# vshmyhlo/retinanet-tensorflow

Measured on AMD Instinct MI355X. Metric: train images/sec (MobileNetV2-FPN RetinaNet 512x512, bs=2/GPU), higher is better.
Workload: dtype f32

## Files before the change

### include/rn_hip.h

```cpp
#ifndef RN_HIP_H
#define RN_HIP_H

#include <stddef.h>
#include <stdint.h>

#ifdef __cplusplus
extern "C" {
#endif

typedef void* rn_stream_t;

enum rn_status {
  RN_OK = 0,
  RN_EINVAL = -1,
  RN_EUNSUPPORTED = -2,
  RN_EHIP = -3,
  RN_EWORKSPACE = -4
};

enum rn_act { RN_ACT_NONE = 0, RN_ACT_RELU = 1, RN_ACT_ELU = 2, RN_ACT_RELU6 = 3, RN_ACT_SIGMOID = 4 };
enum rn_loss_mode { RN_LOSS_BCE_DICE = 0, RN_LOSS_FOCAL = 1 };
enum rn_opt { RN_OPT_MOMENTUM = 0, RN_OPT_RMSPROP = 1, RN_OPT_ADAM = 2 };

#define RN_MAX_SEG 16

typedef struct rn_reduce_list rn_reduce_list;

#define RN_API_VERSION 411
int rn_version(void);
const char* rn_last_error(void);

void rn_same_pad(int n, int k, int s, int* out, int* pad_before);

typedef struct rn_conv_seg {
  const float* x;
  const float* wgt;
  const float* bias;
  float* y;
  const float* dy;
  float* dx;
  int32_t n, h, w;
  int32_t cout;
  int32_t x_ld;
  int32_t x_coff;
  int64_t wgt_bytes;
} rn_conv_seg;

typedef struct rn_conv_geom {
  int32_t kh, kw, stride, cin;
  int32_t groups;
} rn_conv_geom;
// ... 220 lines not shown

size_t rn_resize_pair_u8_augment_batch_workspace(int k, int oh, int ow);
int rn_resize_pair_u8_augment_batch(const uint8_t* raw, int64_t sample_stride_bytes, const rn_augment_desc* desc, int k,
                                    float* pairs, int oh, int ow, const float* mean, const float* stdv, void* workspace,
                                    size_t workspace_bytes, rn_stream_t stream);

typedef struct rn_loss_seg {
  const float* cls_logit;
  const float* cls_label;
  const float* reg_pred;
  const float* reg_label;
  const uint8_t* trainable;
  float* d_cls_logit;
  float* d_reg_pred;
  int64_t rows;
} rn_loss_seg;

#define RN_LOSS_STATS_HEADER 8
size_t rn_loss_workspace(const rn_loss_seg* segs, int nseg, int num_classes);
int rn_loss_fwd(const rn_loss_seg* segs, int nseg, int num_classes, int mode, float* stats, float* class_loss_out,
                float* regr_loss_out, void* workspace, size_t workspace_bytes, rn_stream_t stream);
int rn_loss_bwd(const rn_loss_seg* segs, int nseg, int num_classes, int mode, const float* stats,
                const float* g_cls, const float* g_reg, rn_stream_t stream);

typedef struct rn_wino_gn {
  const float* in_rows;
  const float* in_gamma;
  const float* in_beta;
  int32_t in_groups, in_act;
  float in_eps;
  float* out_rows;
  int32_t out_groups;
  const void* u_ready;
  int32_t urot_ready;
} rn_wino_gn;
size_t rn_wino_gn_rows(const rn_conv_seg* segs, int nseg, int tile);
size_t rn_conv3x3_winograd_gn_u_bytes(int cin, int cout, int tile);
int rn_conv3x3_winograd_gn_weights(const float* w, int cin, int cout, int tile, void* u_out, size_t u_out_bytes, float* urot_out,
                                   rn_stream_t stream);
int rn_conv3x3_winograd_gn(const rn_conv_seg* segs, int nseg, int cin, int cout, const float* w, const float* bias, int tile,
                           const rn_wino_gn* gn, void* workspace, size_t workspace_bytes, float* v_buf, float* urot_buf,
                           rn_stream_t stream);
typedef struct rn_wino_gn_bwd {
  const float* in_rows;
  const float* in_gamma;
  const float* in_beta;
// ... 182 lines not shown
```

### retinanet-tensorflow_amd/_rn.py

```python
import ctypes as C
import os

import torch

_HERE = os.path.dirname(os.path.abspath(__file__))
LIB_PATH = os.environ.get("RN_LIB_PATH") or os.path.join(_HERE, "librn_hip.so")

MAX_SEG = 16
ACT = {None: 0, "none": 0, "linear": 0, "relu": 1, "elu": 2, "relu6": 3, "sigmoid": 4}
LOSS_MODE = {"bce_dice": 0, "focal": 1}
OPT = {"momentum": 0, "rmsprop": 1, "adam": 2}
OPT_BLOCK = 1024
LR_MAX_BOUNDARIES = 8
LOSS_STATS_HEADER = 8
API_VERSION = 411


class RnError(RuntimeError):
    pass


class LrSchedule(C.Structure):
    _fields_ = [("kind", C.c_int32), ("n_boundaries", C.c_int32), ("base_lr", C.c_double), ("warmup_factor", C.c_double),
                ("final_factor", C.c_double), ("decay_factor", C.c_double), ("warmup_steps", C.c_int64), ("total_steps", C.c_int64),
                ("boundaries", C.c_int64 * LR_MAX_BOUNDARIES)]


class ConvSeg(C.Structure):
    _fields_ = [("x", C.c_void_p), ("wgt", C.c_void_p), ("bias", C.c_void_p), ("y", C.c_void_p),
                ("dy", C.c_void_p), ("dx", C.c_void_p),
                ("n", C.c_int32), ("h", C.c_int32), ("w", C.c_int32), ("cout", C.c_int32),
                ("x_ld", C.c_int32), ("x_coff", C.c_int32), ("wgt_bytes", C.c_int64)]


class AssignLevel(C.Structure):
    _fields_ = [("anchor_sizes", C.c_void_p), ("grid_h", C.c_int32), ("grid_w", C.c_int32), ("cls_out", C.c_void_p),
                ("reg_out", C.c_void_p), ("trainable_out", C.c_void_p), ("argmax_out", C.c_void_p)]

# ... 112 lines not shown
class DetParams(C.Structure):
    _fields_ = [("n", C.c_int32), ("num_classes", C.c_int32), ("max_per_class", C.c_int32),
                ("score_threshold", C.c_float), ("iou_threshold", C.c_float), ("max_candidates", C.c_int64)]


_lib = None

SYMBOLS = [
    "rn_version", "rn_last_error", "rn_same_pad",
    "rn_conv2d_fwd_workspace", "rn_conv2d_dgrad_workspace",
    "rn_zero", "rn_conv2d_fwd", "rn_conv2d_stats_rows", "rn_conv2d_fwd_stats", "rn_conv2d_dropout_rows", "rn_conv2d_fwd_dropout", "rn_depthwise_stats_rows", "rn_depthwise_fwd_stats", "rn_group_norm_rows_ok",
    "rn_conv2d_dgrad", "rn_conv2d_wgrad_workspace", "rn_conv2d_wgrad", "rn_conv2d_bwd",
    "rn_conv2d_bias_grad_workspace", "rn_conv2d_bias_grad", "rn_conv3x3_winograd_workspace", "rn_conv3x3_winograd",
    "rn_conv3x3_winograd_wgrad_workspace", "rn_conv3x3_winograd_wgrad", "rn_conv3x3_winograd_keep_bytes",
    "rn_conv3x3_winograd_bwd_workspace", "rn_conv3x3_winograd_bwd", "rn_flush_reductions", "rn_gemm_batched",
    "rn_winograd_bwd_products_workspace", "rn_winograd_bwd_products", "rn_wino_gn_rows", "rn_conv3x3_winograd_gn", "rn_conv3x3_winograd_gn_bwd", "rn_conv3x3_winograd_gn_bwd_wgrad", "rn_reduce_rows", "rn_resize_bilinear_normalize", "rn_resize_pair_u8",
    "rn_resize_pair_u8_augment_workspace", "rn_resize_pair_u8_augment",
    "rn_resize_pair_u8_batch", "rn_resize_pair_u8_augment_batch_workspace", "rn_resize_pair_u8_augment_batch",
    "rn_dwgn_supported", "rn_dwgn_fwd", "rn_dwgn_bwd", "rn_depthwise_fwd", "rn_depthwise_dgrad", "rn_depthwise_wgrad_workspace", "rn_depthwise_wgrad", "rn_depthwise_bwd",
    "rn_group_norm_sync_bytes", "rn_group_norm_workspace", "rn_group_norm_fwd", "rn_group_norm_bwd",
    "rn_act_fwd", "rn_act_bwd", "rn_upsample_add_fwd", "rn_upsample_add_bwd_top",
    "rn_pack_weights_f16", "rn_pack_weights_f16_bytes", "rn_cast_f32_to_f16", "rn_pad_cast_rgb_f16", "rn_conv2d_fwd_f16", "rn_conv2d_f16_fold_rows", "rn_conv2d_fwd_f16_fold", "rn_group_norm_finalize", "rn_group_norm_apply_f16", "rn_group_norm_apply_res_f16", "rn_maxpool_fwd_f16", "rn_maxpool_gn_fwd_f16", "rn_upsample_add_fwd_f16",
    "rn_act_fwd_f16", "rn_flip_width", "rn_dropout", "rn_dropout_strided", "rn_maxpool_fwd", "rn_maxpool_bwd", "rn_maxpool_bwd_arg", "rn_avgpool_fwd", "rn_avgpool_bwd",
    "rn_loss_workspace", "rn_loss_fwd", "rn_loss_bwd",
    "rn_iou", "rn_anchor_assign", "rn_anchor_assign_levels", "rn_anchor_assign_levels_pair", "rn_decode_boxes", "rn_detect_workspace", "rn_detect",
    "rn_boxes_decode", "rn_nms_classwise_workspace", "rn_nms_classwise",
    "rn_optimizer_workspace", "rn_grad_norm_l2reg", "rn_optimizer_step", "rn_counter_add", "rn_add_segs",
    "rn_mb_rows_max", "rn_mb_compact_rows_layout", "rn_mb_compact_rows", "rn_mb_pointwise_rows", "rn_mb_pointwise_fwd", "rn_mb_depthwise_rows", "rn_mb_depthwise_fwd", "rn_mb_apply",
    "rn_mb_resident_sync_bytes", "rn_mb_resident_rows", "rn_mb_resident_fwd", "rn_set_product_mode", "rn_get_product_mode",
    "rn_set_x3_bfrag", "rn_get_x3_bfrag", "rn_x3_bfrag_ok", "rn_x3_bfrag_bytes", "rn_x3_pack_bfrag", "rn_gemm_batched_bfrag", "rn_conv3x3_winograd_gn_u_bytes", "rn_conv3x3_winograd_gn_weights",
    "rn_conv2d_f16_stats_tiles", "rn_group_norm_fwd_f16_tiles",
    "rn_mb_pointwise_bwd_rows", "rn_mb_pointwise_bwd_workspace", "rn_mb_pointwise_bwd",
    "rn_mb_depthwise_bwd_rows", "rn_mb_depthwise_bwd_workspace", "rn_mb_depthwise_bwd",
    "rn_debug_collective_standin", "rn_optimizer_norm_pairs", "rn_optimizer_step_norm", "rn_norm_reg_finalize",
    "rn_lr_schedule_eval", "rn_optimizer_step_norm_lrdev",
]


def lib():
    global _lib
    if _lib is None:
        if not os.path.exists(LIB_PATH):
            raise RnError("librn_hip.so not found at %s: build it with "
                          "`make -C retinanet-tensorflow_amd/csrc` (there is no fallback path)" % LIB_PATH)
        L = C.CDLL(LIB_PATH)
        if not hasattr(L, "rn_version") or L.rn_version() != API_VERSION:
            raise RnError("%s reports ABI version %s, these bindings need %d: rebuild it (make -C retinanet-tensorflow_amd/csrc)"
# ... 110 lines not shown
        L.rn_conv2d_fwd_f16_fold.argtypes = [C.c_void_p, C.c_int, C.c_void_p, C.c_void_p, C.c_void_p]
        L.rn_group_norm_finalize.argtypes = [C.c_void_p, C.c_int, C.c_int, C.c_int, C.c_int, C.c_int, C.c_float, C.c_void_p, C.c_void_p, C.c_void_p]
        L.rn_group_norm_apply_f16.argtypes = [C.c_void_p, C.c_void_p, C.c_void_p, C.c_int, C.c_int, C.c_int, C.c_int, C.c_void_p, C.c_void_p,
                                              C.c_void_p, C.c_void_p, C.c_int, C.c_int, C.c_void_p]
        L.rn_group_norm_apply_res_f16.argtypes = [C.c_void_p, C.c_void_p, C.c_void_p, C.c_void_p, C.c_int, C.c_int, C.c_int, C.c_int, C.c_void_p,
                                                  C.c_void_p, C.c_void_p, C.c_void_p, C.c_int, C.c_int, C.c_void_p]
        L.rn_maxpool_fwd_f16.argtypes = [C.c_void_p] * 2 + [C.c_int] * 6 + [C.c_void_p]
        L.rn_maxpool_gn_fwd_f16.argtypes = [C.c_void_p] * 2 + [C.c_int] * 6 + [C.c_void_p] * 4 + [C.c_int] * 2 + [C.c_void_p]
        L.rn_upsample_add_fwd_f16.argtypes = [C.c_void_p] * 3 + [C.c_int] * 6 + [C.c_void_p]
        L.rn_act_fwd_f16.argtypes = [C.c_void_p, C.c_void_p, C.c_int64, C.c_int, C.c_void_p]
        L.rn_flip_width.argtypes = [C.c_void_p, C.c_void_p, C.c_int64, C.c_int, C.c_int64, C.c_int, C.c_int, C.c_int, C.c_void_p]
        L.rn_dropout_strided.argtypes = [C.c_void_p, C.c_void_p, C.c_int64] + [C.c_int] * 5 + [C.c_float, C.c_uint64, C.c_void_p, C.c_void_p]
        L.rn_dropout.argtypes = [C.c_void_p, C.c_void_p, C.c_int64, C.c_float, C.c_uint64, C.c_void_p, C.c_void_p]
        L.rn_maxpool_fwd.argtypes = [C.c_void_p] * 3 + [C.c_int] * 6 + [C.c_void_p]
        L.rn_maxpool_bwd_arg.argtypes = [C.c_void_p] * 3 + [C.c_int] * 6 + [C.c_void_p]
        L.rn_maxpool_bwd.argtypes = [C.c_void_p] * 3 + [C.c_int] * 6 + [C.c_void_p]
        L.rn_avgpool_fwd.argtypes = [C.c_void_p] * 2 + [C.c_int] * 6 + [C.c_void_p]
        L.rn_avgpool_bwd.argtypes = [C.c_void_p] * 2 + [C.c_int] * 6 + [C.c_void_p]
        L.rn_loss_workspace.argtypes = [C.c_void_p, C.c_int, C.c_int]
        L.rn_loss_fwd.argtypes = [C.c_void_p, C.c_int, C.c_int, C.c_int, C.c_void_p, C.c_void_p, C.c_void_p, C.c_void_p, C.c_size_t,
                                  C.c_void_p]
        L.rn_loss_bwd.argtypes = [C.c_void_p, C.c_int, C.c_int, C.c_int, C.c_void_p, C.c_void_p, C.c_void_p,
                                  C.c_void_p]
        L.rn_iou.argtypes = [C.c_void_p, C.c_int64, C.c_void_p, C.c_int64, C.c_int, C.c_void_p, C.c_void_p, C.c_void_p]
        L.rn_anchor_assign.argtypes = [C.c_void_p] * 3 + [C.c_int, C.c_int, C.c_void_p] + [C.c_int] * 4 + \
                                      [C.c_void_p] * 4 + [C.c_void_p]
        L.rn_anchor_assign_levels.argtypes = [C.c_void_p] * 3 + [C.c_int, C.c_int, C.c_void_p, C.c_int, C.c_int, C.c_int,
                                              C.c_void_p]
        L.rn_anchor_assign_levels_pair.argtypes = L.rn_anchor_assign_levels.argtypes
        L.rn_decode_boxes.argtypes = [C.c_void_p] * 3 + [C.c_int] * 4 + [C.c_void_p]
        L.rn_detect_workspace.argtypes = [C.c_void_p, C.c_int, C.c_void_p]
        L.rn_detect.argtypes = [C.c_void_p, C.c_int, C.c_void_p] + [C.c_void_p] * 6 + [C.c_void_p, C.c_size_t,
                                                                                     C.c_void_p]
        L.rn_boxes_decode.argtypes = L.rn_detect.argtypes
        L.rn_nms_classwise_workspace.argtypes = [C.c_void_p]
        L.rn_nms_classwise.argtypes = [C.c_void_p] * 5 + [C.c_void_p] + [C.c_void_p] * 6 + [C.c_void_p, C.c_size_t,
                                                                                        C.c_void_p]
        L.rn_grad_norm_l2reg.argtypes = [C.c_void_p] * 3 + [C.c_int64, C.c_float, C.c_void_p, C.c_void_p,
                                                             C.c_size_t, C.c_void_p]
        L.rn_optimizer_step.argtypes = [C.c_int] + [C.c_void_p] * 5 + [C.c_int64, C.c_float, C.c_float,
                                                                       C.c_float, C.c_void_p, C.c_int64,
                                                                       C.c_void_p, C.c_uint64, C.c_void_p]
        L.rn_counter_add.argtypes = [C.c_void_p, C.c_uint64, C.c_void_p]
        L.rn_add_segs.argtypes = [C.c_void_p, C.c_int, C.c_void_p]
        for name in ("rn_mb_pointwise_rows", "rn_mb_depthwise_rows", "rn_mb_pointwise_bwd_rows", "rn_mb_pointwise_bwd_workspace",
                     "rn_mb_depthwise_bwd_rows", "rn_mb_depthwise_bwd_workspace"):
# ... 173 lines not shown
```

### retinanet-tensorflow_amd/csrc/loss.hip

```cpp
#include "rn_common.h"

namespace {

constexpr int T = 256;
constexpr int WAVES = T / 64;
constexpr int MAXJ = 4;
constexpr int NSCAL = 5;
constexpr int BLOCKS = 2048;

struct LossSeg {
  const float* zl; const float* ll; const float* rp; const float* rl; const uint8_t* tm;
  float* dz; float* dr;
  int64_t rows; int64_t row_start;
};
struct LossArgs {
  LossSeg seg[RN_MAX_SEG];
  int nseg, C, mode;
  int64_t total_rows;
  float* partial;
  float* stats;
  float* cls_out; float* reg_out;
  const float* g_cls; const float* g_reg;
};

__device__ __forceinline__ int seg_of_row(const LossArgs& a, int64_t r) {
  int s = 0;
  while (s + 1 < a.nseg && r >= a.seg[s + 1].row_start) ++s;
  return s;
}
__device__ __forceinline__ float sigmoidf(float z) { return 1.f / (1.f + expf(-z)); }
__device__ __forceinline__ float clip1(float e) { return e < -1.f ? -1.f : (e > 1.f ? 1.f : e); }
__device__ __forceinline__ float huber1(float e) {
  const float a = fabsf(e), q = fminf(a, 1.f);
  return 0.5f * q * q + (a - q);
}

__global__ __launch_bounds__(T) void loss_reduce_kernel(const LossArgs a) {
  __shared__ float red[WAVES][NSCAL + 3 * 64 * MAXJ];
  const int tid = threadIdx.x, lane = tid & 63, wave = tid >> 6;
  const int C = a.C;
  float I[MAXJ], L[MAXJ], P[MAXJ];
#pragma unroll
  for (int j = 0; j < MAXJ; ++j) I[j] = L[j] = P[j] = 0.f;
  float s_m = 0.f, s_fg = 0.f, s_bce = 0.f, s_focal = 0.f, s_hub = 0.f;

// ... 202 lines not shown
          if (MODE == RN_LOSS_BCE_DICE) {
            const float U = Uc[k][e];
            g[e] = k_bce * (p - lv) - k_dice * p * (1.f - p) * (lv * U - Ic[k][e]) / (U * U);
          } else {
            const bool pos = (lv == 1.f);
            const float pt = pos ? p : 1.f - p;
            const float al = pos ? 0.25f : 0.75f;
            const float om = 1.f - pt;
            const float dfdpt = -al * (-2.f * om * logf(pt + 1e-7f) + om * om / (pt + 1e-7f));
            g[e] = k_focal * dfdpt * (pos ? 1.f : -1.f) * p * (1.f - p);
          }
          g[e] = tmv[u] != 0.f ? g[e] : 0.f;
        }
        if (live[u] && j + 4 * k < CQ) *reinterpret_cast<float4*>(dzp[u] + (j + 4 * k) * 4) = make_float4(g[0], g[1], g[2], g[3]);
      }
      lmax = fmaxf(lmax, __shfl_xor(lmax, 1, 64));
      lmax = fmaxf(lmax, __shfl_xor(lmax, 2, 64));
      if (live[u]) {
        float g = 0.f;
        if (tmv[u] != 0.f) g = ((lmax > 0.5f) ? 1.f : 0.f) * (k_reg * clip1(rp[u] - rl[u]));
        *drp[u] = g;
      }
    }
  }
}

__global__ __launch_bounds__(256) void loss_sum_kernel(const LossArgs a, int nblocks, double* __restrict__ sums) {
  __shared__ double sh[16][16];
  const int n = NSCAL + 3 * a.C;
  const int il = threadIdx.x & 15, rl = threadIdx.x >> 4;
  const int i = blockIdx.x * 16 + il;
  double v = 0.0;
  if (i < n) {
    int b = rl;
    for (; b + 16 * 7 < nblocks; b += 16 * 8) {
      float t[8];
#pragma unroll
      for (int u = 0; u < 8; ++u) t[u] = a.partial[(size_t)(b + 16 * u) * n + i];
#pragma unroll
      for (int u = 0; u < 8; ++u) v += (double)t[u];
    }
    for (; b < nblocks; b += 16) v += (double)a.partial[(size_t)b * n + i];
  }
  sh[rl][il] = v;
  __syncthreads();
  if (rl == 0 && i < n) {
// ... 130 lines not shown
    if (mode == RN_LOSS_BCE_DICE) hipLaunchKernelGGL((loss_reduce4_kernel<NK, RN_LOSS_BCE_DICE>), grid, block, 0, st, a);
    else hipLaunchKernelGGL((loss_reduce4_kernel<NK, RN_LOSS_FOCAL>), grid, block, 0, st, a);
  } else {
    if (mode == RN_LOSS_BCE_DICE) hipLaunchKernelGGL((loss_grad4_kernel<NK, RN_LOSS_BCE_DICE>), grid, block, 0, st, a);
    else hipLaunchKernelGGL((loss_grad4_kernel<NK, RN_LOSS_FOCAL>), grid, block, 0, st, a);
  }
}
template <bool REDUCE>
bool launch4(const LossArgs& a, int C, int mode, hipStream_t st) {
  if (!use4(C)) return false;
  switch ((C / 4 + 3) / 4) {
    case 1: launch4_nk<REDUCE, 1>(a, mode, st); break;
    case 2: launch4_nk<REDUCE, 2>(a, mode, st); break;
    case 3: launch4_nk<REDUCE, 3>(a, mode, st); break;
    case 4: launch4_nk<REDUCE, 4>(a, mode, st); break;
    case 5: launch4_nk<REDUCE, 5>(a, mode, st); break;
    case 6: launch4_nk<REDUCE, 6>(a, mode, st); break;
    case 7: launch4_nk<REDUCE, 7>(a, mode, st); break;
    default: launch4_nk<REDUCE, 8>(a, mode, st); break;
  }
  return true;
}

int nblocks_for(int64_t rows) {
  int64_t b = (rows + WAVES * 4 - 1) / (WAVES * 4);
  if (b > BLOCKS) b = BLOCKS;
  if (b < 1) b = 1;
  return (int)b;
}
}

extern "C" size_t rn_loss_workspace(const rn_loss_seg*, int, int num_classes) {
  return rn::align_up((size_t)BLOCKS * (NSCAL + 3 * (size_t)num_classes) * sizeof(float), 256) +
         (NSCAL + 3 * (size_t)num_classes) * sizeof(double);
}

extern "C" int rn_loss_fwd(const rn_loss_seg* segs, int nseg, int num_classes, int mode, float* stats, float* class_loss_out,
                           float* regr_loss_out, void* workspace, size_t workspace_bytes, rn_stream_t stream) {
  LossArgs a = {};
  if (int e = build(segs, nseg, num_classes, mode, &a, false)) return e;
  RN_CHECK_ARG(stats && workspace, "loss fwd: null stats/workspace");
  if (workspace_bytes < rn_loss_workspace(segs, nseg, num_classes)) {
    rn::set_error("loss fwd: workspace too small");
    return RN_EWORKSPACE;
  }
  a.partial = (float*)workspace; a.stats = stats; a.cls_out = class_loss_out; a.reg_out = regr_loss_out;
  hipStream_t st = (hipStream_t)stream;
  const int nb = use4(num_classes) ? nblocks4(a.total_rows) : nblocks_for(a.total_rows);
  if (!launch4<true>(a, num_classes, mode, st)) hipLaunchKernelGGL(loss_reduce_kernel, dim3(nb), dim3(T), 0, st, a);
  double* sums = (double*)((char*)workspace + rn::align_up((size_t)BLOCKS * (NSCAL + 3 * (size_t)num_classes) * sizeof(float), 256));
  hipLaunchKernelGGL(loss_sum_kernel, dim3(rn::ceil_div(NSCAL + 3 * num_classes, 16)), dim3(256), 0, st, a, nb, sums);
  hipLaunchKernelGGL(loss_finalize_kernel, dim3(1), dim3(256), 0, st, a, (const double*)sums);
  RN_LAUNCH_CHECK();
  return RN_OK;
}

extern "C" int rn_loss_bwd(const rn_loss_seg* segs, int nseg, int num_classes, int mode, const float* stats,
                           const float* g_cls, const float* g_reg, rn_stream_t stream) {
  LossArgs a = {};
  if (int e = build(segs, nseg, num_classes, mode, &a, true)) return e;
  RN_CHECK_ARG(stats && g_cls && g_reg, "loss bwd: null stats/upstream gradient");
  a.stats = const_cast<float*>(stats); a.g_cls = g_cls; a.g_reg = g_reg;
  if (!launch4<false>(a, num_classes, mode, (hipStream_t)stream))
    hipLaunchKernelGGL(loss_grad_kernel, dim3(nblocks_for(a.total_rows)), dim3(T), 0, (hipStream_t)stream, a);
  RN_LAUNCH_CHECK();
  return RN_OK;
}
```

### retinanet-tensorflow_amd/losses.py

```python
import ops

LOSS_MODE = 'bce_dice'


def loss(labels, logits, trainable_masks=None, mode=None, name='loss', return_stats=False):
    mode = mode or LOSS_MODE
    keys = list(logits.regression.keys())
    if trainable_masks is None:
        trainable_masks = getattr(labels, 'trainable_masks', None)
    if trainable_masks is None:
        raise AssertionError('losses.loss needs trainable_masks (dict P3..P7 of [N,H,W,A] uint8/bool)')
    cls_logits = [logits.classification.unscaled[k] for k in keys]
    num_classes = cls_logits[0].shape[-1]
    class_loss, regr_loss, stats = ops.detection_loss(
        cls_logits, [logits.regression[k] for k in keys],
        [labels.classification.prob[k] for k in keys], [labels.regression[k] for k in keys],
        [trainable_masks[k] for k in keys], num_classes, mode)
    if return_stats:
        return class_loss, regr_loss, stats
    return class_loss, regr_loss
```

### retinanet-tensorflow_amd/ops.py

```python
import ctypes as C
import os

import torch

import _rn


DIRECT_PARAM_GRADS = False


WGRAD_SIDE_STREAM = False


class _on_side_stream(object):

    def __init__(self, device, tensors, direct=True):
        self.on = WGRAD_SIDE_STREAM and direct and device.type == 'cuda'
        if self.on:
            self.side = _rn.side_stream(device, 0)
            self.side.wait_stream(torch.cuda.current_stream(device))
            for t in tensors:
                if t is not None:
                    t.record_stream(self.side)
            self.ctx = torch.cuda.stream(self.side)
# ... 974 lines not shown
    def backward(ctx, g_cls, g_reg, _g_stats):
        n = ctx.n
        saved = ctx.saved_tensors
        stats = saved[0]
        cls_logits = list(saved[1:1 + n])
        reg_preds = list(saved[1 + n:1 + 2 * n])
        cls_labels = list(saved[1 + 2 * n:1 + 3 * n])
        reg_labels = list(saved[1 + 3 * n:1 + 4 * n])
        masks = list(saved[1 + 4 * n:1 + 5 * n])
        dev = stats.device
        zero = None
        if g_cls is None or g_reg is None:
            zero = torch.zeros((1,), dtype=torch.float32, device=dev)
        g_cls = g_cls.reshape(1).contiguous().float() if g_cls is not None else zero
        g_reg = g_reg.reshape(1).contiguous().float() if g_reg is not None else zero
        dcls = [torch.empty_like(z) for z in cls_logits]
        dreg = [torch.empty_like(r) for r in reg_preds]
        segs = _loss_segs(cls_logits, cls_labels, reg_preds, reg_labels, masks, dcls, dreg)
        _rn.check(_rn.lib().rn_loss_bwd(segs, n, ctx.num_classes, _rn.LOSS_MODE[ctx.mode], _rn.f32(stats),
                                        _rn.f32(g_cls), _rn.f32(g_reg), _rn.stream()), "rn_loss_bwd")
        return (None, None, None) + tuple(dcls) + tuple(dreg) + (None,) * (3 * n)


def detection_loss(cls_logits, reg_preds, cls_labels, reg_labels, trainable_masks, num_classes, mode="bce_dice"):
    n = len(cls_logits)
    return _DetectionLoss.apply(mode, num_classes, n, *cls_logits, *reg_preds, *cls_labels, *reg_labels,
                                *trainable_masks)


class _Dropout(torch.autograd.Function):

    @staticmethod
    def forward(ctx, x, rate, seed, seed_dev):
        x = x.contiguous()
        y = torch.empty_like(x)
        _rn.check(_rn.lib().rn_dropout(_rn.f32(x), _rn.f32(y), x.numel(), rate, seed,
                                       seed_dev.data_ptr() if seed_dev is not None else None, _rn.stream()), "rn_dropout")
        ctx.cfg = (rate, seed, seed_dev)
        return y

    @staticmethod
    def backward(ctx, dy):
        rate, seed, seed_dev = ctx.cfg
        dy = dy.contiguous()
        dx = torch.empty_like(dy)
        _rn.check(_rn.lib().rn_dropout(_rn.f32(dy), _rn.f32(dx), dy.numel(), rate, seed,
                                       seed_dev.data_ptr() if seed_dev is not None else None, _rn.stream()), "rn_dropout")
        return dx, None, None, None
# ... 297 lines not shown
```

### retinanet-tensorflow_amd/train.py

```python
import collections
import contextlib
import ctypes
import math
import os
import sys
import time

import numpy as np
import torch

import _rn
import layers as L
import losses
import ops
import utils
from levels import build_levels

OPT_BLOCK = _rn.OPT_BLOCK
FUSED_OPT_NORM = os.environ.get("RN_FUSED_OPT_NORM", "1") == "1"


class ParamArena(object):

    def __init__(self, model, device):
# ... 332 lines not shown
        if base is not None and hasattr(base, 'classification_subnet'):
            first = next(iter(base.classification_subnet.parameters()), None)
            self.heads_offset = self._param_offset.get(id(first), self.arena.count)
        self.whole_step_graph = os.environ.get("RN_WHOLE_STEP_GRAPH", "1") == "1"
        if capture_collectives is False:
            self.allreduce._capturable = False
        if self.allreduce.active and use_graph and self.whole_step_graph and self.device.type == 'cuda':
            self.allreduce.probe_capturable(self.device)
        self.defer_wgrad = os.environ.get("RN_DEFER_WGRAD", "1") == "1" and self.device.type == 'cuda' and self.direct_param_grads
        self.wino_pre = os.environ.get("RN_WINO_PRE", "0") == "1" and self.device.type == 'cuda'
        self._wino_pre = None
        self._deferred_wgrads = []
        self._deferred_running = []
        self._graphs = None
        self._graph_cache = collections.OrderedDict()
        self.graph_cache_max = max(1, int(os.environ.get("RN_GRAPH_CACHE", "4")))
        self.schedule = []
        self._last_lr, self._lr_changes = None, 0
        self.recaptures = 0
        self._static = None
        self.drop_rank_offset = self.allreduce.rank * 0x632BE59BD9B4E019 % (1 << 62)
        self.drop_counter = torch.full((1,), self.drop_rank_offset, dtype=torch.int64, device=self.device)
        self._one = torch.ones((), dtype=torch.float32, device=self.device)
        self.check_interval = int(check_interval)
        self.steps_done = 0
        self.timing = None
        self.last = {}

    @contextlib.contextmanager
    def _scoped(self):
        saved = (ops.DIRECT_PARAM_GRADS, ops.WGRAD_SIDE_STREAM, L.Dropout.seed_device_counter)
        ops.DIRECT_PARAM_GRADS, ops.WGRAD_SIDE_STREAM = self.direct_param_grads, self.wgrad_side_stream
        L.Dropout.seed_device_counter = self.drop_counter
        base = self._cut_base
        saved_cut = base.backward_cut if base is not None else None
        saved_stage = self._stage_bb.stage_cut if self._stage_bb is not None else None
        if base is not None:
            base.backward_cut = self._cut
        if self._stage_bb is not None:
            self._stage_bb.stage_cut = self._stage_cut
        try:
            yield
        finally:
            ops.DIRECT_PARAM_GRADS, ops.WGRAD_SIDE_STREAM, L.Dropout.seed_device_counter = saved
            if base is not None:
                base.backward_cut = saved_cut
# ... 36 lines not shown

    def _backward(self, roots, grads, skip_join=()):
        defer = self.defer_reductions and self.device.type == 'cuda' and ops.DIRECT_PARAM_GRADS
        if defer:
            import retinanet
            extra = [retinanet.side_stream(self.device)] if retinanet.HEADS_TWO_STREAMS else []
            if ops.WGRAD_SIDE_STREAM:
                extra.append(_rn.side_stream(self.device, 0))
            if os.environ.get("RN_DEFER_SIDE", "1") != "1":
                extra = []
            ops.begin_deferred_reductions(extra)
        try:
            torch.autograd.backward(roots, grads)
        finally:
            if defer:
                ops.end_deferred_reductions()
        if self.device.type == 'cuda':
            _rn.join_side_streams(self.device, skip=skip_join)

    def segment_a(self, features=None):
        with self._scoped():
            label_stream = None
            zeroed = False
            if features is None:
                if self.device.type == 'cuda' and getattr(self.input_fn, 'concurrent', False):
                    label_stream = _rn.side_stream(self.device, 2)
                    label_stream.wait_stream(torch.cuda.current_stream())
                    main_stream = torch.cuda.current_stream()
                    with torch.cuda.stream(label_stream):
                        features = self.input_fn()
                        self.arena.zero_grad()
                        zeroed = True
                    _for_each_tensor(features, lambda t: t.record_stream(main_stream) if t.is_cuda else None)
                else:
                    features = self.input_fn()
            self._cut_src = self._cut_leaves = None
            self._stage_cuts = []
            self._parts = []
            ops.begin_direct_grad_step()
            pre_ev = self._fork_kernel_transforms()
            try:
                logits = {'detection': self.net(features['image'], training=True)}
            finally:
                ops.WINO_PRE = {}
            if pre_ev is not None:
                torch.cuda.current_stream().wait_event(pre_ev)
            if label_stream is not None:
                torch.cuda.current_stream().wait_stream(label_stream)
            inp, logits = utils.process_labels_and_logits(labels=features, logits=logits, levels=self.levels)
            class_loss, regr_loss = losses.loss(labels=inp['detection_trainable'], logits=logits['detection_trainable'],
                                                mode=self.loss_mode)
            if not zeroed:
                self.arena.zero_grad()
            ops.WGRAD_DEFER = [] if self.defer_wgrad else None
            try:
                self._backward([class_loss, regr_loss], [self._one, self._one])
            finally:
                self._deferred_wgrads, ops.WGRAD_DEFER = (ops.WGRAD_DEFER or []), None
            if self._cut_src is not None:
                self._parts = self._plan_parts()
                self._cut_src = self._cut_leaves = None
                self._stage_cuts = []
            if self._deferred_wgrads and not self._parts:
                ops.run_deferred_wgrads(self._deferred_wgrads)
                self._deferred_wgrads = []
            return class_loss.detach(), regr_loss.detach()

    PRE_STREAM = 8

    def _fork_kernel_transforms(self):
        if not self.wino_pre or not (ops.WINO_GN_FOLD and ops.WINOGRAD):
            return None
        if self._wino_pre is None:
            if torch.cuda.is_current_stream_capturing():
                return None
            base = getattr(self.net, 'base', self.net)
            subnets = [getattr(base, n, None) for n in ('classification_subnet', 'regression_subnet')]
            kernels = [w for sn in subnets if sn is not None and hasattr(sn, 'tower_kernels') for w in sn.tower_kernels()]
            if not kernels:
                return None
            self._wino_pre = ops.WinoPretransform(kernels)
        side = _rn.side_stream(self.device, self.PRE_STREAM)
        side.wait_stream(torch.cuda.current_stream())
        with torch.cuda.stream(side):
            ops.WINO_PRE, ev = self._wino_pre.launch()
        return ev

    def num_parts(self):
        return len(self._parts)
# ... 19 lines not shown
                    _rn.check(_rn.lib().rn_gemm_batched(_rn.f32(A_), _rn.f32(B_), _rn.f32(C_), A_.shape[1], 256, 256, 36, 0, _rn.stream()), "rn_gemm_batched")
        if self._deferred_wgrads:
            self._fork_wgrads(after_wgrads)
        skip = () if join_wgrads else (self.WGRAD_STREAM,)
        for j in (range(len(self._parts)) if part is None else [part]):
            roots, seeds, rng = self._parts[j]
            with self._scoped():
                self._backward(roots, [l.grad for l in seeds], skip_join=skip)
        if side is not None:
            torch.cuda.current_stream().wait_stream(side)
        if part is None:
            self._parts = []
            return (0, self.cut_offset)
        return rng

    def _fork_wgrads(self, after=None):
        if self.device.type == 'cuda':
            wside = _rn.side_stream(self.device, self.WGRAD_STREAM)
            wside.wait_stream(torch.cuda.current_stream())
            with torch.cuda.stream(wside):
                ops.run_deferred_wgrads(self._deferred_wgrads)
                if after is not None:
                    after()
        else:
            ops.run_deferred_wgrads(self._deferred_wgrads)
            if after is not None:
                after()
        self._deferred_running = self._deferred_wgrads
        self._deferred_wgrads = []

    def _join_wgrads(self):
        if self.device.type == 'cuda':
            torch.cuda.current_stream().wait_stream(_rn.side_stream(self.device, self.WGRAD_STREAM))

    def forward_backward(self, features=None, advance_dropout=True):
        out = self.segment_a(features)
        self.segment_b()
        if advance_dropout and self.device.type == 'cuda':
            ops.advance_dropout_counter(self.drop_counter)
        return out

    def _run_step(self, features=None, timed=False):
        ar = self.allreduce
        del self.schedule[:]

        def reduce(lo, hi):
            if hi > lo:
                self.schedule.append((lo, hi))
                ar.launch(lo, hi)

# ... 495 lines not shown
```

Baseline: 485.6.

## Fuse focal loss forward and backward into one pass using precomputed label counts

```diff
diff --git a/include/rn_hip.h b/include/rn_hip.h
--- a/include/rn_hip.h
+++ b/include/rn_hip.h
@@ -26,7 +26,7 @@
 
 typedef struct rn_reduce_list rn_reduce_list;
 
-#define RN_API_VERSION 411
+#define RN_API_VERSION 412
 int rn_version(void);
 const char* rn_last_error(void);
 
@@ -293,6 +293,13 @@
                 float* regr_loss_out, void* workspace, size_t workspace_bytes, rn_stream_t stream);
 int rn_loss_bwd(const rn_loss_seg* segs, int nseg, int num_classes, int mode, const float* stats,
                 const float* g_cls, const float* g_reg, rn_stream_t stream);
+
+#define RN_LOSS_COUNTS_FLOATS (2 + 2 * 2048)
+int rn_loss_counts(const rn_loss_seg* segs, int nseg, int num_classes, float* counts, rn_stream_t stream);
+int rn_loss_fwd_bwd(const rn_loss_seg* segs, int nseg, int num_classes, int mode, const float* counts, const float* g_cls,
+                    const float* g_reg, void* partial, size_t partial_bytes, rn_stream_t stream);
+int rn_loss_finalize(int64_t total_rows, int num_classes, int mode, float* stats, float* class_loss_out, float* regr_loss_out,
+                     void* partial, size_t partial_bytes, rn_stream_t stream);
 
 typedef struct rn_wino_gn {
   const float* in_rows;
diff --git a/retinanet-tensorflow_amd/_rn.py b/retinanet-tensorflow_amd/_rn.py
--- a/retinanet-tensorflow_amd/_rn.py
+++ b/retinanet-tensorflow_amd/_rn.py
@@ -13,7 +13,8 @@
 OPT_BLOCK = 1024
 LR_MAX_BOUNDARIES = 8
 LOSS_STATS_HEADER = 8
-API_VERSION = 411
+LOSS_COUNTS_FLOATS = 2 + 2 * 2048
+API_VERSION = 412
 
 
 class RnError(RuntimeError):
@@ -172,7 +173,7 @@
     "rn_act_fwd", "rn_act_bwd", "rn_upsample_add_fwd", "rn_upsample_add_bwd_top",
     "rn_pack_weights_f16", "rn_pack_weights_f16_bytes", "rn_cast_f32_to_f16", "rn_pad_cast_rgb_f16", "rn_conv2d_fwd_f16", "rn_conv2d_f16_fold_rows", "rn_conv2d_fwd_f16_fold", "rn_group_norm_finalize", "rn_group_norm_apply_f16", "rn_group_norm_apply_res_f16", "rn_maxpool_fwd_f16", "rn_maxpool_gn_fwd_f16", "rn_upsample_add_fwd_f16",
     "rn_act_fwd_f16", "rn_flip_width", "rn_dropout", "rn_dropout_strided", "rn_maxpool_fwd", "rn_maxpool_bwd", "rn_maxpool_bwd_arg", "rn_avgpool_fwd", "rn_avgpool_bwd",
-    "rn_loss_workspace", "rn_loss_fwd", "rn_loss_bwd",
+    "rn_loss_workspace", "rn_loss_fwd", "rn_loss_bwd", "rn_loss_counts", "rn_loss_fwd_bwd", "rn_loss_finalize",
     "rn_iou", "rn_anchor_assign", "rn_anchor_assign_levels", "rn_anchor_assign_levels_pair", "rn_decode_boxes", "rn_detect_workspace", "rn_detect",
     "rn_boxes_decode", "rn_nms_classwise_workspace", "rn_nms_classwise",
     "rn_optimizer_workspace", "rn_grad_norm_l2reg", "rn_optimizer_step", "rn_counter_add", "rn_add_segs",
@@ -329,6 +330,11 @@
                                   C.c_void_p]
         L.rn_loss_bwd.argtypes = [C.c_void_p, C.c_int, C.c_int, C.c_int, C.c_void_p, C.c_void_p, C.c_void_p,
                                   C.c_void_p]
+        L.rn_loss_counts.argtypes = [C.c_void_p, C.c_int, C.c_int, C.c_void_p, C.c_void_p]
+        L.rn_loss_fwd_bwd.argtypes = [C.c_void_p, C.c_int, C.c_int, C.c_int, C.c_void_p, C.c_void_p, C.c_void_p, C.c_void_p, C.c_size_t,
+                                      C.c_void_p]
+        L.rn_loss_finalize.argtypes = [C.c_int64, C.c_int, C.c_int, C.c_void_p, C.c_void_p, C.c_void_p, C.c_void_p, C.c_size_t,
+                                       C.c_void_p]
         L.rn_iou.argtypes = [C.c_void_p, C.c_int64, C.c_void_p, C.c_int64, C.c_int, C.c_void_p, C.c_void_p, C.c_void_p]
         L.rn_anchor_assign.argtypes = [C.c_void_p] * 3 + [C.c_int, C.c_int, C.c_void_p] + [C.c_int] * 4 + \
                                       [C.c_void_p] * 4 + [C.c_void_p]
diff --git a/retinanet-tensorflow_amd/csrc/loss.hip b/retinanet-tensorflow_amd/csrc/loss.hip
--- a/retinanet-tensorflow_amd/csrc/loss.hip
+++ b/retinanet-tensorflow_amd/csrc/loss.hip
@@ -21,6 +21,7 @@
   float* stats;
   float* cls_out; float* reg_out;
   const float* g_cls; const float* g_reg;
+  const float* counts;
 };
 
 __device__ __forceinline__ int seg_of_row(const LossArgs& a, int64_t r) {
@@ -269,6 +270,141 @@
         *drp[u] = g;
       }
     }
+  }
+}
+
+__global__ __launch_bounds__(T) void loss_count_kernel(const LossArgs a, float* __restrict__ part) {
+  __shared__ float red[WAVES][2];
+  const int tid = threadIdx.x, lane = tid & 63, wave = tid >> 6;
+  const int C = a.C, CQ = C >> 2, j = lane & 3, r16 = lane >> 2;
+  float s_m = 0.f, s_fg = 0.f;
+  const int64_t ngroups = (a.total_rows + RPW - 1) / RPW;
+  const int64_t wave_id = (int64_t)blockIdx.x * WAVES + wave, nwaves = (int64_t)gridDim.x * WAVES;
+  for (int64_t g0 = wave_id; g0 < ngroups; g0 += nwaves) {
+    const int64_t r = g0 * RPW + r16;
+    float lmax = -1e30f, tmv = 0.f;
+    if (r < a.total_rows) {
+      const LossSeg& sg = a.seg[seg_of_row(a, r)];
+      const int64_t lr = r - sg.row_start;
+      tmv = sg.tm[lr] ? 1.f : 0.f;
+      if (tmv != 0.f) {
+        for (int q = j; q < CQ; q += 4) {
+          const float4 l = *reinterpret_cast<const float4*>(sg.ll + lr * C + q * 4);
+          lmax = fmaxf(lmax, fmaxf(fmaxf(l.x, l.y), fmaxf(l.z, l.w)));
+        }
+      }
+    }
+    lmax = fmaxf(lmax, __shfl_xor(lmax, 1, 64));
+    lmax = fmaxf(lmax, __shfl_xor(lmax, 2, 64));
+    if (j == 0) { s_m += tmv; s_fg += (lmax > 0.5f) ? tmv : 0.f; }
+  }
+  s_m = rn::wave_sum(s_m); s_fg = rn::wave_sum(s_fg);
+  if (lane == 0) { red[wave][0] = s_m; red[wave][1] = s_fg; }
+  __syncthreads();
+  if (tid < 2) {
+    float v = 0.f;
+#pragma unroll
+    for (int w = 0; w < WAVES; ++w) v += red[w][tid];
+    part[2 * blockIdx.x + tid] = v;
+  }
+}
+
+__global__ __launch_bounds__(256) void loss_count_finalize_kernel(const float* __restrict__ part, int nblocks, float* __restrict__ counts) {
+  __shared__ double sh[2][128];
+  const int i = threadIdx.x & 1, t = threadIdx.x >> 1;
+  double v = 0.0;
+  for (int b = t; b < nblocks; b += 128) v += (double)part[2 * b + i];
+  sh[i][t] = v;
+  __syncthreads();
+  if (threadIdx.x < 2) {
+    double s = 0.0;
+    for (int u = 0; u < 128; ++u) s += sh[threadIdx.x][u];
+    counts[threadIdx.x] = (float)s;
+  }
+}
+
+template <int NK>
+__global__ __launch_bounds__(T) void loss_fwd_bwd4_kernel(const LossArgs a) {
+  __shared__ float red[WAVES][NSCAL];
+  const int tid = threadIdx.x, lane = tid & 63, wave = tid >> 6;
+  const int C = a.C, CQ = C >> 2, j = lane & 3, r16 = lane >> 2;
+  const float nfg = a.counts[1];
+  const float gc = a.g_cls[0], gr = a.g_reg[0];
+  const float k_focal = gc / fmaxf(nfg, 1.f);
+  const float k_reg = nfg > 0.f ? gr / (4.f * nfg) : 0.f;
+  float s_m = 0.f, s_fg = 0.f, s_cls = 0.f, s_hub = 0.f;
+  const int64_t ngroups = (a.total_rows + RPW - 1) / RPW;
+  const int64_t wave_id = (int64_t)blockIdx.x * WAVES + wave, nwaves = (int64_t)gridDim.x * WAVES;
+  for (int64_t g0 = wave_id * 2; g0 < ngroups; g0 += nwaves * 2) {
+    float4 z[2][NK], l[2][NK];
+    float rl[2], rp[2], tmv[2];
+    float* dzp[2]; float* drp[2]; bool live[2];
+#pragma unroll
+    for (int u = 0; u < 2; ++u) {
+      const int64_t r = min((g0 + u) * RPW + r16, a.total_rows - 1);
+      live[u] = (g0 + u) * RPW + r16 < a.total_rows;
+      const LossSeg& sg = a.seg[seg_of_row(a, r)];
+      const int64_t lr = r - sg.row_start;
+      tmv[u] = (live[u] && sg.tm[lr]) ? 1.f : 0.f;
+      rl[u] = sg.rl[lr * 4 + j]; rp[u] = sg.rp[lr * 4 + j];
+      dzp[u] = sg.dz + lr * C; drp[u] = sg.dr + lr * 4 + j;
+#pragma unroll
+      for (int k = 0; k < NK; ++k) {
+        const int q = min(j + 4 * k, CQ - 1);
+        z[u][k] = *reinterpret_cast<const float4*>(sg.zl + lr * C + q * 4);
+        l[u][k] = *reinterpret_cast<const float4*>(sg.ll + lr * C + q * 4);
+      }
+    }
+#pragma unroll
+    for (int u = 0; u < 2; ++u) {
+      float lmax = -1e30f, cls = 0.f;
+#pragma unroll
+      for (int k = 0; k < NK; ++k) {
+        const float w = (j + 4 * k < CQ) ? tmv[u] : 0.f;
+        const float zz[4] = {z[u][k].x, z[u][k].y, z[u][k].z, z[u][k].w}, ll[4] = {l[u][k].x, l[u][k].y, l[u][k].z, l[u][k].w};
+        float g[4];
+#pragma unroll
+        for (int e = 0; e < 4; ++e) {
+          const float zv = zz[e], lv = ll[e];
+          const float p = sigmoidf(zv);
+          if (j + 4 * k < CQ) lmax = fmaxf(lmax, lv);
+          const bool pos = (lv == 1.f);
+          const float pt = pos ? p : 1.f - p;
+          const float al = pos ? 0.25f : 0.75f;
+          const float om = 1.f - pt;
+          cls = fmaf(w, -al * om * om * logf(pt + 1e-7f), cls);
+          const float dfdpt = -al * (-2.f * om * logf(pt + 1e-7f) + om * om / (pt + 1e-7f));
+          g[e] = k_focal * dfdpt * (pos ? 1.f : -1.f) * p * (1.f - p);
+          g[e] = tmv[u] != 0.f ? g[e] : 0.f;
+        }
+        if (live[u] && j + 4 * k < CQ) *reinterpret_cast<float4*>(dzp[u] + (j + 4 * k) * 4) = make_float4(g[0], g[1], g[2], g[3]);
+      }
+      lmax = fmaxf(lmax, __shfl_xor(lmax, 1, 64));
+      lmax = fmaxf(lmax, __shfl_xor(lmax, 2, 64));
+      const float fgw = (lmax > 0.5f) ? 1.f : 0.f;
+      const float fg = fgw * tmv[u];
+      s_cls += cls;
+      if (j == 0) { s_m += tmv[u]; s_fg += fg; }
+      const float hub = fgw * huber1(rl[u] - rp[u]);
+      s_hub += (tmv[u] != 0.f) ? hub : 0.f;
+      if (live[u]) {
+        float g = 0.f;
+        if (tmv[u] != 0.f) g = ((lmax > 0.5f) ? 1.f : 0.f) * (k_reg * clip1(rp[u] - rl[u]));
+        *drp[u] = g;
+      }
+    }
+  }
+  s_m = rn::wave_sum(s_m); s_fg = rn::wave_sum(s_fg); s_cls = rn::wave_sum(s_cls); s_hub = rn::wave_sum(s_hub);
+  if (lane == 0) { red[wave][0] = s_m; red[wave][1] = s_fg; red[wave][2] = 0.f; red[wave][3] = s_cls; red[wave][4] = s_hub; }
+  __syncthreads();
+  const int n = NSCAL + 3 * C;
+  for (int i = tid; i < n; i += T) {
+    float v = 0.f;
+    if (i < NSCAL) {
+#pragma unroll
+      for (int w = 0; w < WAVES; ++w) v += red[w][i];
+    }
+    a.partial[(size_t)blockIdx.x * n + i] = v;
   }
 }
 
@@ -445,6 +581,13 @@
   return true;
 }
 
+template <int NK>
+void launch_fwd_bwd4(const LossArgs& a, hipStream_t st) {
+  hipLaunchKernelGGL((loss_fwd_bwd4_kernel<NK>), dim3(nblocks4(a.total_rows)), dim3(T), 0, st, a);
+}
+bool one_pass_ok(int C, int mode) { return mode == RN_LOSS_FOCAL && use4(C); }
+size_t partial_bytes(int C) { return rn::align_up((size_t)BLOCKS * (NSCAL + 3 * (size_t)C) * sizeof(float), 256); }
+
 int nblocks_for(int64_t rows) {
   int64_t b = (rows + WAVES * 4 - 1) / (WAVES * 4);
   if (b > BLOCKS) b = BLOCKS;
@@ -489,3 +632,74 @@
   RN_LAUNCH_CHECK();
   return RN_OK;
 }
+
+extern "C" int rn_loss_counts(const rn_loss_seg* segs, int nseg, int num_classes, float* counts, rn_stream_t stream) {
+  RN_CHECK_ARG(segs && nseg >= 1 && nseg <= RN_MAX_SEG, "loss counts: bad segments");
+  RN_CHECK_ARG(counts, "loss counts: null counts");
+  RN_UNSUPPORTED(num_classes < 4 || num_classes > 128 || num_classes % 4 != 0,
+                 "loss counts: num_classes %d is not a multiple of 4 in [4,128]", num_classes);
+  LossArgs a = {};
+  a.nseg = nseg; a.C = num_classes; a.mode = RN_LOSS_FOCAL;
+  int64_t rows = 0;
+  for (int s = 0; s < nseg; ++s) {
+    RN_CHECK_ARG(segs[s].cls_label && segs[s].trainable && segs[s].rows >= 0, "loss counts: null pointer in segment %d", s);
+    a.seg[s].ll = segs[s].cls_label; a.seg[s].tm = segs[s].trainable; a.seg[s].rows = segs[s].rows; a.seg[s].row_start = rows;
+    rows += segs[s].rows;
+  }
+  a.total_rows = rows;
+  int64_t nb = (rows + RPW * WAVES - 1) / (RPW * WAVES);
+  if (nb > BLOCKS) nb = BLOCKS;
+  if (nb < 1) nb = 1;
+  hipStream_t st = (hipStream_t)stream;
+  hipLaunchKernelGGL(loss_count_kernel, dim3((int)nb), dim3(T), 0, st, a, counts + 2);
+  hipLaunchKernelGGL(loss_count_finalize_kernel, dim3(1), dim3(256), 0, st, (const float*)(counts + 2), (int)nb, counts);
+  RN_LAUNCH_CHECK();
+  return RN_OK;
+}
+
+extern "C" int rn_loss_fwd_bwd(const rn_loss_seg* segs, int nseg, int num_classes, int mode, const float* counts, const float* g_cls,
+                               const float* g_reg, void* partial, size_t partial_bytes_, rn_stream_t stream) {
+  LossArgs a = {};
+  if (int e = build(segs, nseg, num_classes, mode, &a, true)) return e;
+  RN_UNSUPPORTED(!one_pass_ok(num_classes, mode), "loss fwd+bwd: one pass covers focal mode with num_classes %% 4 == 0 in [4,128] (got %d, mode %d)",
+                 num_classes, mode);
+  RN_CHECK_ARG(counts && g_cls && g_reg && partial, "loss fwd+bwd: null counts/upstream gradient/partial");
+  if (partial_bytes_ < rn_loss_workspace(segs, nseg, num_classes)) {
+    rn::set_error("loss fwd+bwd: partial buffer too small");
+    return RN_EWORKSPACE;
+  }
+  a.partial = (float*)partial; a.counts = counts; a.g_cls = g_cls; a.g_reg = g_reg;
+  hipStream_t st = (hipStream_t)stream;
+  switch ((num_classes / 4 + 3) / 4) {
+    case 1: launch_fwd_bwd4<1>(a, st); break;
+    case 2: launch_fwd_bwd4<2>(a, st); break;
+    case 3: launch_fwd_bwd4<3>(a, st); break;
+    case 4: launch_fwd_bwd4<4>(a, st); break;
+    case 5: launch_fwd_bwd4<5>(a, st); break;
+    case 6: launch_fwd_bwd4<6>(a, st); break;
+    case 7: launch_fwd_bwd4<7>(a, st); break;
+    default: launch_fwd_bwd4<8>(a, st); break;
+  }
+  RN_LAUNCH_CHECK();
+  return RN_OK;
+}
+
+extern "C" int rn_loss_finalize(int64_t total_rows, int num_classes, int mode, float* stats, float* class_loss_out, float* regr_loss_out,
+                                void* partial, size_t partial_bytes_, rn_stream_t stream) {
+  RN_UNSUPPORTED(!one_pass_ok(num_classes, mode), "loss finalize: one pass covers focal mode with num_classes %% 4 == 0 in [4,128] (got %d, mode %d)",
+                 num_classes, mode);
+  RN_CHECK_ARG(stats && partial && total_rows >= 0, "loss finalize: null stats/partial");
+  if (partial_bytes_ < rn_loss_workspace(nullptr, 0, num_classes)) {
+    rn::set_error("loss finalize: partial buffer too small");
+    return RN_EWORKSPACE;
+  }
+  LossArgs a = {};
+  a.C = num_classes; a.mode = mode; a.total_rows = total_rows;
+  a.partial = (float*)partial; a.stats = stats; a.cls_out = class_loss_out; a.reg_out = regr_loss_out;
+  hipStream_t st = (hipStream_t)stream;
+  double* sums = (double*)((char*)partial + partial_bytes(num_classes));
+  hipLaunchKernelGGL(loss_sum_kernel, dim3(rn::ceil_div(NSCAL + 3 * num_classes, 16)), dim3(256), 0, st, a, nblocks4(total_rows), sums);
+  hipLaunchKernelGGL(loss_finalize_kernel, dim3(1), dim3(256), 0, st, a, (const double*)sums);
+  RN_LAUNCH_CHECK();
+  return RN_OK;
+}
diff --git a/retinanet-tensorflow_amd/losses.py b/retinanet-tensorflow_amd/losses.py
--- a/retinanet-tensorflow_amd/losses.py
+++ b/retinanet-tensorflow_amd/losses.py
@@ -3,7 +3,7 @@
 LOSS_MODE = 'bce_dice'
 
 
-def loss(labels, logits, trainable_masks=None, mode=None, name='loss', return_stats=False):
+def loss(labels, logits, trainable_masks=None, mode=None, name='loss', return_stats=False, counts=None, seeds=None):
     mode = mode or LOSS_MODE
     keys = list(logits.regression.keys())
     if trainable_masks is None:
@@ -15,7 +15,23 @@
     class_loss, regr_loss, stats = ops.detection_loss(
         cls_logits, [logits.regression[k] for k in keys],
         [labels.classification.prob[k] for k in keys], [labels.regression[k] for k in keys],
-        [trainable_masks[k] for k in keys], num_classes, mode)
+        [trainable_masks[k] for k in keys], num_classes, mode, counts=counts, seeds=seeds)
     if return_stats:
         return class_loss, regr_loss, stats
     return class_loss, regr_loss
+
+
+def loss_counts(labels, trainable_masks, mode=None, out=None):
+    keys = list(labels.keys())
+    num_classes = labels[keys[0]].shape[-1]
+    if not ops.loss_one_pass_ok(num_classes, mode or LOSS_MODE):
+        return None
+    return ops.detection_loss_counts([labels[k] for k in keys], [trainable_masks[k] for k in keys], num_classes, out=out)
+
+
+def finish():
+    return ops.finish_detection_loss()
+
+
+def abandon():
+    del ops._loss_pending[:]
diff --git a/retinanet-tensorflow_amd/ops.py b/retinanet-tensorflow_amd/ops.py
--- a/retinanet-tensorflow_amd/ops.py
+++ b/retinanet-tensorflow_amd/ops.py
@@ -1020,8 +1020,93 @@
         return (None, None, None) + tuple(dcls) + tuple(dreg) + (None,) * (3 * n)
 
 
-def detection_loss(cls_logits, reg_preds, cls_labels, reg_labels, trainable_masks, num_classes, mode="bce_dice"):
+LOSS_ONE_PASS = os.environ.get("RN_LOSS_ONE_PASS", "1") != "0"
+_LOSS_WAVE_PER_ROW = bool(int(os.environ.get("RN_LOSS_WAVE_PER_ROW", "0") or 0))
+_loss_pending = []
+
+
+def loss_one_pass_ok(num_classes, mode):
+    return (LOSS_ONE_PASS and not _LOSS_WAVE_PER_ROW and mode == "focal"
+            and num_classes % 4 == 0 and 4 <= num_classes <= 128)
+
+
+def detection_loss_counts(cls_labels, trainable_masks, num_classes, out=None):
+    n = len(cls_labels)
+    labels = [t.contiguous() for t in cls_labels]
+    masks = [t.contiguous() for t in trainable_masks]
+    for l, m in zip(labels, masks):
+        assert m.dtype in (torch.uint8, torch.bool) and l.shape[-1] == num_classes and l.numel() == m.numel() * num_classes
+    if out is None:
+        out = torch.empty((_rn.LOSS_COUNTS_FLOATS,), dtype=torch.float32, device=labels[0].device)
+    assert out.numel() >= _rn.LOSS_COUNTS_FLOATS
+    segs = (_rn.LossSeg * n)()
+    for i in range(n):
+        segs[i].cls_label = _rn.f32(labels[i])
+        segs[i].trainable = _rn.ptr(masks[i])
+        segs[i].rows = masks[i].numel()
+    _rn.check(_rn.lib().rn_loss_counts(segs, n, num_classes, _rn.f32(out), _rn.stream()), "rn_loss_counts")
+    return out
+
+
+class _DetectionLossOnePass(torch.autograd.Function):
+
+    @staticmethod
+    def forward(ctx, num_classes, n, counts, seed_cls, seed_reg, *tensors):
+        cls_logits = [t.contiguous() for t in tensors[:n]]
+        reg_preds = [t.contiguous() for t in tensors[n:2 * n]]
+        cls_labels = [t.contiguous() for t in tensors[2 * n:3 * n]]
+        reg_labels = [t.contiguous() for t in tensors[3 * n:4 * n]]
+        masks = [t.contiguous() for t in tensors[4 * n:5 * n]]
+        for m in masks:
+            assert m.dtype in (torch.uint8, torch.bool)
+        for z, l, m in zip(cls_logits, cls_labels, masks):
+            assert z.shape == l.shape and z.shape[-1] == num_classes and z.numel() == m.numel() * num_classes
+        assert seed_cls.numel() == 1 and seed_reg.numel() == 1
+        L = _rn.lib()
+        dev = cls_logits[0].device
+        stats = torch.empty((_rn.LOSS_STATS_HEADER + 3 * num_classes,), dtype=torch.float32, device=dev)
+        class_loss = torch.empty((), dtype=torch.float32, device=dev)
+        regr_loss = torch.empty((), dtype=torch.float32, device=dev)
+        dcls = [torch.empty_like(z) for z in cls_logits]
+        dreg = [torch.empty_like(r) for r in reg_preds]
+        segs = _loss_segs(cls_logits, cls_labels, reg_preds, reg_labels, masks, dcls, dreg)
+        partial = torch.empty((L.rn_loss_workspace(segs, n, num_classes),), dtype=torch.uint8, device=dev)
+        _rn.check(L.rn_loss_fwd_bwd(segs, n, num_classes, _rn.LOSS_MODE["focal"], _rn.f32(counts), _rn.f32(seed_cls), _rn.f32(seed_reg),
+                                    partial.data_ptr(), partial.numel(), _rn.stream()), "rn_loss_fwd_bwd")
+        rows = sum(m.numel() for m in masks)
+        _loss_pending.append((rows, num_classes, stats, class_loss, regr_loss, partial))
+        ctx.n, ctx.grads, ctx.seeds = n, (dcls, dreg), (seed_cls, seed_reg)
+        ctx.mark_non_differentiable(stats)
+        ctx.set_materialize_grads(False)
+        return class_loss, regr_loss, stats
+
+    @staticmethod
+    def backward(ctx, g_cls, g_reg, _g_stats):
+        for g, seed in zip((g_cls, g_reg), ctx.seeds):
+            if g is None or g.data_ptr() != seed.data_ptr():
+                raise _rn.RnError("one-pass detection loss: backward must be seeded with the tensors handed to detection_loss(seeds=...)")
+        dcls, dreg = ctx.grads
+        ctx.grads = None
+        return (None,) * 5 + tuple(dcls) + tuple(dreg) + (None,) * (3 * ctx.n)
+
+
+def finish_detection_loss():
+    done = []
+    while _loss_pending:
+        rows, num_classes, stats, class_loss, regr_loss, partial = _loss_pending.pop(0)
+        _rn.check(_rn.lib().rn_loss_finalize(rows, num_classes, _rn.LOSS_MODE["focal"], _rn.f32(stats), _rn.f32(class_loss),
+                                             _rn.f32(regr_loss), partial.data_ptr(), partial.numel(), _rn.stream()), "rn_loss_finalize")
+        done.append((stats, class_loss, regr_loss, partial))
+    return done
+
+
+def detection_loss(cls_logits, reg_preds, cls_labels, reg_labels, trainable_masks, num_classes, mode="bce_dice",
+                   counts=None, seeds=None):
     n = len(cls_logits)
+    if (counts is not None and seeds is not None and loss_one_pass_ok(num_classes, mode) and torch.is_grad_enabled()
+            and all(t.requires_grad for t in list(cls_logits) + list(reg_preds))):
+        return _DetectionLossOnePass.apply(num_classes, n, counts, seeds[0], seeds[1], *cls_logits, *reg_preds, *cls_labels,
+                                           *reg_labels, *trainable_masks)
     return _DetectionLoss.apply(mode, num_classes, n, *cls_logits, *reg_preds, *cls_labels, *reg_labels,
                                 *trainable_masks)
 
diff --git a/retinanet-tensorflow_amd/train.py b/retinanet-tensorflow_amd/train.py
--- a/retinanet-tensorflow_amd/train.py
+++ b/retinanet-tensorflow_amd/train.py
@@ -378,6 +378,8 @@
         self.drop_rank_offset = self.allreduce.rank * 0x632BE59BD9B4E019 % (1 << 62)
         self.drop_counter = torch.full((1,), self.drop_rank_offset, dtype=torch.int64, device=self.device)
         self._one = torch.ones((), dtype=torch.float32, device=self.device)
+        self._loss_counts = None
+        self._loss_running = []
         self.check_interval = int(check_interval)
         self.steps_done = 0
         self.timing = None
@@ -460,6 +462,7 @@
         with self._scoped():
             label_stream = None
             zeroed = False
+            counts = None
             if features is None:
                 if self.device.type == 'cuda' and getattr(self.input_fn, 'concurrent', False):
                     label_stream = _rn.side_stream(self.device, 2)
@@ -467,6 +470,7 @@
                     main_stream = torch.cuda.current_stream()
                     with torch.cuda.stream(label_stream):
                         features = self.input_fn()
+                        counts = self._label_counts(features)
                         self.arena.zero_grad()
                         zeroed = True
                     _for_each_tensor(features, lambda t: t.record_stream(main_stream) if t.is_cuda else None)
@@ -475,6 +479,7 @@
             self._cut_src = self._cut_leaves = None
             self._stage_cuts = []
             self._parts = []
+            losses.abandon()
             ops.begin_direct_grad_step()
             pre_ev = self._fork_kernel_transforms()
             try:
@@ -485,9 +490,11 @@
                 torch.cuda.current_stream().wait_event(pre_ev)
             if label_stream is not None:
                 torch.cuda.current_stream().wait_stream(label_stream)
+            if counts is None:
+                counts = self._label_counts(features)
             inp, logits = utils.process_labels_and_logits(labels=features, logits=logits, levels=self.levels)
             class_loss, regr_loss = losses.loss(labels=inp['detection_trainable'], logits=logits['detection_trainable'],
-                                                mode=self.loss_mode)
+                                                mode=self.loss_mode, counts=counts, seeds=(self._one, self._one))
             if not zeroed:
                 self.arena.zero_grad()
             ops.WGRAD_DEFER = [] if self.defer_wgrad else None
@@ -502,7 +509,17 @@
             if self._deferred_wgrads and not self._parts:
                 ops.run_deferred_wgrads(self._deferred_wgrads)
                 self._deferred_wgrads = []
+            if not (self._deferred_wgrads and self._parts):
+                self._loss_running = losses.finish()
             return class_loss.detach(), regr_loss.detach()
+
+    def _label_counts(self, features):
+        if self.device.type != 'cuda':
+            return None
+        labels = features['detection']['classifications']
+        if self._loss_counts is None:
+            self._loss_counts = torch.zeros(_rn.LOSS_COUNTS_FLOATS, dtype=torch.float32, device=self.device)
+        return losses.loss_counts(labels, features['trainable_masks'], mode=self.loss_mode, out=self._loss_counts)
 
     PRE_STREAM = 8
 
@@ -568,10 +585,12 @@
                 ops.run_deferred_wgrads(self._deferred_wgrads)
                 if after is not None:
                     after()
+                self._loss_running = losses.finish()
         else:
             ops.run_deferred_wgrads(self._deferred_wgrads)
             if after is not None:
                 after()
+            self._loss_running = losses.finish()
         self._deferred_running = self._deferred_wgrads
         self._deferred_wgrads = []
 
```

Measured after the change: 483.5. No clear change (-0.4%).
